# AniruddhaMandal/SS-GNN

Measured on AMD Instinct MI355X. Metric: k_subgraphs_sampled_per_sec, higher is better.
Workload: dtype int64; 1 GPU; c5_er_1m; graphs=1, columns=19999981, k=8, rows_per_gpu=1000000, global_rows=1000000, mode=sample, collate=none (single GPU)

## Files before the change

### include/ugs_mi355.h

```cpp
#ifndef UGS_MI355_H
#define UGS_MI355_H

#include <stdint.h>

#ifdef __cplusplus
extern "C" {
#endif

#define UGS_OK 0
#define UGS_E_INVALID_HANDLE (-1)
#define UGS_E_NO_ROOTS (-2)
#define UGS_E_BAD_MODE (-3)
#define UGS_E_BAD_ARG (-4)
#define UGS_E_NO_DEVICE (-5)
#define UGS_E_HIP (-6)
#define UGS_E_UNSUPPORTED (-7)
#define UGS_E_EDGE_SRC (-8)
#define UGS_E_CAPACITY (-9)

#define UGS_EDGE_LOCAL 0
#define UGS_EDGE_FLAT 1
#define UGS_EDGE_GLOBAL 2
#define UGS_MODE_SAMPLE 0
#define UGS_MODE_GRAPH 1
// ... 37 lines not shown
int ugs_sample_batch_stream(const int64_t *edge_index, int64_t row_stride, int64_t num_cols, const int64_t *ptr,
                            int64_t num_graphs, int m_per_graph, int k, int mode, int seed, int64_t edge_capacity,
                            int64_t *nodes, int64_t *edge_index_out, int64_t *edge_ptr, int64_t *sample_ptr,
                            int64_t *edge_src_global, int64_t *total_edges_out);
int ugs_sample_stream(int64_t handle, int m_per_graph, int k, int edge_mode, int64_t base_offset, int seed,
                      int64_t edge_capacity, int64_t *nodes, int64_t *edge_index_out, int64_t *edge_ptr, int64_t *edge_src,
                      int64_t *total_edges_out);
int ugs_stream_stats(int64_t *early_starts_kept, int64_t *early_starts_discarded);

int ugs_cache_clear(void);
int ugs_cache_stats(int64_t *size, int64_t *hits, int64_t *misses);
int ugs_batch_pass_stats(int64_t *device_plans, int64_t *general_path);
int ugs_set_batch_pass_max_cols(int64_t cols, int64_t *previous_out);
int64_t ugs_batch_pass_max_cols(void);

typedef struct ugs_plan ugs_plan;
int ugs_plan_create_batch(const int64_t *edge_index, int64_t row_stride, int64_t num_cols, const int64_t *ptr,
                          int64_t num_graphs, int k, ugs_plan **plan_out);
int ugs_plan_create_handle(int64_t handle, ugs_plan **plan_out);
int ugs_plan_release(ugs_plan *plan);
int ugs_plan_graph_roots(ugs_plan *plan, int64_t graph, int64_t capacity, int32_t *level, int32_t *num_nodes, int32_t *num_viable,
                         double *prob, int32_t *alias, int32_t *v_self, int32_t *v_alias, int32_t *viable_vi, int32_t *viable_v);
int ugs_plan_twin(ugs_plan *plan, int k, ugs_plan **twin_out);
int ugs_plan_info(const ugs_plan *plan, int k, int64_t *num_graphs, int64_t *num_vertices, int64_t *nnz,
                  int64_t *device_bytes, int *tier);
int ugs_plan_walk(ugs_plan *plan, int m_per_graph, int k, int mode, int64_t extra_node_offset, int seed,
                  int64_t row_begin, int64_t row_count, void *stream, int64_t *d_nodes, int64_t *d_edge_ptr,
                  int64_t *total_edges_host);
int ugs_plan_fill(ugs_plan *plan, int m_per_graph, int k, int mode, int64_t extra_node_offset, int64_t row_begin,
                  int64_t row_count, void *stream, const int64_t *d_nodes, const int64_t *d_edge_ptr,
                  int64_t *d_edge_index, int64_t ld, int64_t *d_edge_src);
int ugs_plan_step(ugs_plan *plan, int m_per_graph, int k, int mode, int64_t extra_node_offset, int seed, int64_t row_begin,
                  int64_t row_count, void *stream, int64_t *d_nodes, int64_t *d_edge_ptr, int64_t *d_edge_index, int64_t ld,
                  int64_t *d_edge_src);
int ugs_plan_set_walk_share(ugs_plan *plan, int percent);
typedef struct ugs_graph ugs_graph;
int ugs_plan_graph_create(ugs_plan *plan, int m_per_graph, int k, int mode, int64_t extra_node_offset, int64_t row_begin,
                          int64_t row_count, int64_t *d_nodes, int64_t *d_edge_ptr, int64_t *d_edge_index, int64_t ld,
                          int64_t *d_edge_src, ugs_graph **graph_out);
int ugs_plan_graph_launch(ugs_graph *graph, int seed, void *stream);
int ugs_plan_graph_destroy(ugs_graph *graph);
int ugs_plan_last_launch(const ugs_plan *plan, char *name_buf, int name_buf_len, int *grid, int *block,
                         int *lds_bytes, int64_t *overflow_rows);

int ugs_collate_layout(int k, int node_bytes, int eidx_bytes, int esrc_bytes, int64_t rows_cap, int64_t edge_cap,
                       int64_t *section_off4, int64_t *msg_bytes);
// ... 62 lines not shown
```

### ss-gnn_amd/csrc/ugs_device.h

```cpp
#pragma once
#include <hip/hip_runtime.h>
#include <stdint.h>

#define UGS_KMAX 32

struct UgsGraphDesc {
    int64_t node_lo;
    int64_t rbase;
    int64_t vbase;
    int64_t viable_base;
    int32_t n;
    int32_t level;
    int32_t n_viable;
    int32_t pad;
};

struct UgsRootRec {
    double prob;
    int32_t alias;
    int32_t v_self;
    int32_t v_alias;
    int32_t pad;
};

struct UgsPlanDev {
    const UgsGraphDesc *graphs;
    const int64_t *rowptr;
    const int2 *adj;
    const int2 *adjf;
    const UgsRootRec *roots;
    const int2 *viable;
    int64_t num_graphs;
    const int2 *prow;
    int32_t prow_shift;
    int32_t prow_first;
};

struct UgsWalkArgs {
    UgsPlanDev plan;
    int32_t m;
    int32_t k;
    int32_t mode;
    int32_t pad;
    int64_t extra_node_off;
    uint64_t seed64;
    const uint64_t *seed_ptr;
    int64_t row_begin;
    int64_t row_count;
    int64_t *nodes;
    uint32_t *counts;
    const int64_t *in_list;
    const uint32_t *in_count;
    int64_t *ovf_list;
    uint32_t *ovf_count;
    uint32_t *gws;
    int64_t gws_words_per_group;
    int64_t gws_groups;
    int32_t gcap;
// ... 31 lines not shown
    int64_t *h_total;
    uint32_t *h_flag;
    uint32_t epoch;
};

struct UgsLaunchInfo {
    const char *name;
    int grid, block, lds_bytes;
};

enum { UGS_TIER_S = 0 , UGS_TIER_M = 1 , UGS_TIER_W = 2 ,
       UGS_TIER_X = 3 , UGS_TIER_V = 4 , UGS_TIER_L = 5 ,
       UGS_TIER_G = 6  };
#define UGS_LDS_TIERS 6
static constexpr int UGS_TIER_CAP[UGS_LDS_TIERS] = {64, 448, 704, 1024, 1408, 2048};
static constexpr int UGS_TIER_LANES[UGS_LDS_TIERS] = {8, 64, 64, 64, 64, 64};
static constexpr int UGS_TIER_HASH_LIMIT[UGS_LDS_TIERS] = {96, 448, 896, 1536, 1792, 3072};
#define UGS_SMALL_CAP 32
#define UGS_WIDE_LANES 16
#define UGS_SMALL_HASH_LIMIT 48

hipError_t ugs_launch_walk(const UgsWalkArgs &a, int tier, int device_cus, int share_percent, hipStream_t s, UgsLaunchInfo *info);
hipError_t ugs_launch_build_prow(const UgsPlanDev &plan, int64_t num_vertices, int2 *prow, int shift, int device_cus, hipStream_t s);
#define UGS_COLLATE_MAX_WORLD 64
hipError_t ugs_launch_collate_unpack(const void *d_msgs, int world, int64_t msg_bytes, const int64_t *row_off, int k, int node_b, int eidx_b,
                                     int esrc_b, int64_t rows_cap, int64_t edge_cap, const int64_t *section_off4, int64_t *d_nodes,
                                     int64_t *d_edge_index, int64_t ld, int64_t *d_edge_ptr, int64_t *d_edge_src, int64_t *d_max_total,
                                     hipStream_t s);
hipError_t ugs_launch_rebase_edge_ptr(const int64_t *in, int64_t *out, int64_t n, int64_t base, hipStream_t s);
#define UGS_BATCH_PASS_MAX_COLS 1000
#define UGS_BATCH_PASS_COLS_CEIL 8192
#define UGS_BATCH_PASS_MAX_N 2048
#define UGS_BATCH_PASS_FUSED_WORK (4ll << 20)
int64_t ugs_batch_pass_fused_work();
hipError_t ugs_launch_batch_pass(const int64_t *d_src, const int64_t *d_dst, int64_t E, const int64_t *d_ptr, int64_t G, int k,
                                 int32_t *d_owner, uint32_t *d_cnt_jminc_jmax, const int64_t *d_rstart, int64_t *d_rowptr, int2 *d_adj,
                                 int2 *d_adjf, int32_t *d_vrank, unsigned long long *d_bump, unsigned long long bump_base, uint32_t epoch, void *h_back,
                                 unsigned long long *d_done, unsigned long long done_base, int64_t max_cols, hipStream_t s);
#define UGS_BP_BACK_CNT(G) ((size_t)(G) * 24)
#define UGS_BP_BACK_FLAG(G) ((size_t)(G) * 36)
#define UGS_BP_BACK_BYTES(G) ((size_t)(G) * 36 + 16)
__host__ __device__ inline unsigned long long ugs_fp_mix(unsigned long long x) {
    x ^= x >> 33; x *= 0xff51afd7ed558ccdull; x ^= x >> 33; x *= 0xc4ceb9fe1a85ec53ull; x ^= x >> 33;
    return x;
}
__host__ __device__ inline void ugs_fp_seed(unsigned long long n, unsigned long long cols, unsigned long long &a, unsigned long long &b) {
// ... 105 lines not shown
```

### ss-gnn_amd/csrc/ugs_host.cpp

```cpp
#include "../../include/ugs_mi355.h"
#include "ugs_device.h"

#include <algorithm>
#include <atomic>
#include <cmath>
#include <cstdio>
#include <cstdlib>
#include <cstring>
#include <chrono>
#include <list>
#include <map>
#include <memory>
#include <mutex>
#include <string>
#include <unordered_map>
#include <thread>
#include <vector>

struct ugs_plan;
namespace { void plan_unref(ugs_plan *p); void arena_release(int dev, int64_t roots_off, int64_t n_roots, int64_t via_off, int64_t n_via); void pin_slot_put(char *p); }

struct UgsEpsLaunch {
    const UgsGraphDesc *graphs; const int64_t *rowptr; const int32_t *nbr; const int32_t *ecs; int64_t num_graphs;
    int32_t m, k, mode, max_attempts; uint64_t seed; double epsilon; int64_t rows;
// ... 850 lines not shown
            if (v >= ptr[g] && v < ptr[g + 1]) { owner[(size_t)j] = (int32_t)g; ++cstart[(size_t)g + 1]; }
        }
        for (int64_t g = 0; g < G; ++g) cstart[(size_t)g + 1] += cstart[(size_t)g];
        cols_of.resize((size_t)cstart[(size_t)G]);
        std::vector<int64_t> wr(cstart.begin(), cstart.end() - 1);
        for (int64_t j = 0; j < E; ++j) if (owner[(size_t)j] >= 0) cols_of[(size_t)wr[(size_t)owner[(size_t)j]]++] = j;
    } else {
        for (int64_t g = 0; g < G; ++g) {
            const int64_t lo = ptr[g], hi = ptr[g + 1];
            for (int64_t j = 0; j < E; ++j) if (src[j] >= lo && src[j] < hi && dst[j] >= lo && dst[j] < hi) cols_of.push_back(j);
            cstart[(size_t)g + 1] = (int64_t)cols_of.size();
        }
    }
}

int ensure_prow(ugs_plan *plan, hipStream_t s) {
    if (plan->dev.prow || plan->prow_failed || plan->nverts <= 0) return UGS_OK;
    if (const char *e = std::getenv("UGS_NO_PROW")) if (e[0] == '1') return UGS_OK;
    double sb = 0;
    for (double x : plan->g_sbdeg) sb = std::max(sb, x);
    int shift = 3;
    while (shift < 6 && (double)((1 << shift) - 1) < sb + 3.0 * std::sqrt(sb) + 1.0) ++shift;
    if (const char *e = std::getenv("UGS_PROW_SHIFT")) { const int f = std::atoi(e); if (f >= 3 && f <= 6) shift = f; }
    const size_t bytes = ((size_t)plan->nverts << shift) * sizeof(int2);
    if (bytes >= ((size_t)1 << 32)) { plan->prow_failed = true; return UGS_OK; }
    if (bytes <= ((size_t)64 << 20)) {
        const std::string keep = t_err;
        if (pool_get(bytes, plan->device, plan->prow) != UGS_OK) { t_err = keep; plan->prow_failed = true; return UGS_OK; }
        plan->prow_pooled = true;
    } else {
        void *p = nullptr;
        if (hipMalloc(&p, bytes) != hipSuccess) { (void)hipGetLastError(); plan->prow_failed = true; return UGS_OK; }
        plan->prow.p = p; plan->prow.bytes = bytes; plan->prow.dev = plan->device;
    }
    HIP_TRY(ugs_launch_build_prow(plan->dev, plan->nverts, static_cast<int2 *>(plan->prow.p), shift, plan->cus, s));
    HIP_TRY(hipStreamSynchronize(s));
    plan->dev.prow = static_cast<const int2 *>(plan->prow.p);
    plan->dev.prow_shift = shift;
    int first = (int)std::ceil((sb + 0.5 * std::sqrt(sb) + 1.0) / 16.0) * 16;
    if (const char *e = std::getenv("UGS_PROW_FIRST")) { const int f = std::atoi(e); if (f >= 1) first = f; }
    plan->dev.prow_first = std::max(1, std::min(first, 1 << shift));
    plan->prow_bytes.store(plan->prow.bytes);
    if (plan->cached) plan_cache_trim();
    return UGS_OK;
}

int ensure(PoolBuf &b, size_t bytes, int dev, ugs_plan *plan) {
    if (b.p && b.bytes >= bytes) return UGS_OK;
    if (b.p && plan && plan->last_valid) HIP_TRY(hipEventSynchronize(plan->last_ev));
    pool_put(b);
    return pool_get(bytes, dev, b);
}

bool capturing(hipStream_t s) {
    hipStreamCaptureStatus st = hipStreamCaptureStatusNone;
    return hipStreamIsCapturing(s, &st) == hipSuccess && st != hipStreamCaptureStatusNone;
}
int plan_enter(ugs_plan *plan, hipStream_t s) {
    if (plan->last_valid && plan->last_stream != s && !capturing(s)) HIP_TRY(hipStreamWaitEvent(s, plan->last_ev, 0));
    return UGS_OK;
}
int plan_leave(ugs_plan *plan, hipStream_t s) {
    if (capturing(s)) return UGS_OK;
    if (!plan->last_ev) HIP_TRY(hipEventCreateWithFlags(&plan->last_ev, hipEventDisableTiming));
    HIP_TRY(hipEventRecord(plan->last_ev, s));
// ... 681 lines not shown
        std::lock_guard<std::mutex> lk(plan->mu);
        if (plan->last_valid) HIP_TRY(hipEventSynchronize(plan->last_ev));
        HIP_TRY(hipMemcpy(&d, plan->dev.graphs + graph, sizeof(d), hipMemcpyDeviceToHost));
    }
    if (level) *level = d.level;
    if (num_nodes) *num_nodes = d.n;
    if (num_viable) *num_viable = d.n_viable;
    if (d.level == 0 && d.n > 0 && (prob || alias || v_self || v_alias)) {
        if (capacity < d.n) return fail(UGS_E_BAD_ARG, "capacity below the graph's vertex count");
        std::vector<UgsRootRec> rec((size_t)d.n);
        HIP_TRY(hipMemcpy(rec.data(), plan->dev.roots + d.vbase, rec.size() * sizeof(UgsRootRec), hipMemcpyDeviceToHost));
        for (int32_t vi = 0; vi < d.n; ++vi) {
            if (prob) prob[vi] = rec[(size_t)vi].prob;
            if (alias) alias[vi] = rec[(size_t)vi].alias;
            if (v_self) v_self[vi] = rec[(size_t)vi].v_self;
            if (v_alias) v_alias[vi] = rec[(size_t)vi].v_alias;
        }
    } else if (d.level > 0 && d.n_viable > 0 && (viable_vi || viable_v)) {
        if (capacity < d.n_viable) return fail(UGS_E_BAD_ARG, "capacity below the viable list's length");
        std::vector<int2> v((size_t)d.n_viable);
        HIP_TRY(hipMemcpy(v.data(), plan->dev.viable + d.viable_base, v.size() * sizeof(int2), hipMemcpyDeviceToHost));
        for (int32_t t = 0; t < d.n_viable; ++t) { if (viable_vi) viable_vi[t] = v[(size_t)t].x; if (viable_v) viable_v[t] = v[(size_t)t].y; }
    }
    return UGS_OK;
}

int ugs_plan_info(const ugs_plan *plan, int k, int64_t *num_graphs, int64_t *num_vertices, int64_t *nnz, int64_t *device_bytes, int *tier) {
    if (!plan) return fail(UGS_E_BAD_ARG, "plan is null");
    if (num_graphs) *num_graphs = plan->G;
    if (num_vertices) *num_vertices = plan->nverts;
    if (nnz) *nnz = plan->nnz;
    if (device_bytes) *device_bytes = (int64_t)(plan->blob_bytes + plan->prow.bytes);
    if (tier) *tier = choose_tier(const_cast<ugs_plan *>(plan), k).first;
    return UGS_OK;
}

static int plan_walk_impl(ugs_plan *plan, int m_per_graph, int k, int mode, int64_t extra_node_offset, int seed, const uint64_t *d_seed_ptr,
                          const uint64_t *d_seeds, int64_t row_begin, int64_t row_count, void *stream, int64_t *d_nodes, int64_t *d_edge_ptr, int64_t *total_edges_host,
                          bool *defer_scan = nullptr, bool poll_total = false);
static int plan_walk_locked(ugs_plan *plan, const TierChoice &tc, int m_per_graph, int k, int mode, int64_t extra_node_offset, int seed,
                            const uint64_t *d_seed_ptr, const uint64_t *d_seeds, int64_t row_begin, int64_t row_count, hipStream_t s, int64_t *d_nodes, int64_t *d_edge_ptr,
                            int64_t *total_edges_host, bool *defer_scan, bool poll_total);


int ugs_plan_walk(ugs_plan *plan, int m_per_graph, int k, int mode, int64_t extra_node_offset, int seed, int64_t row_begin,
                  int64_t row_count, void *stream, int64_t *d_nodes, int64_t *d_edge_ptr, int64_t *total_edges_host) {
// ... 1289 lines not shown
```

### ss-gnn_amd/csrc/ugs_kernels.hip

```cpp
#include "ugs_device.h"
#include <cstdlib>

#define UGS_ALIGNED16 __attribute__((aligned(16)))

#ifdef UGS_STAMPS
__device__ unsigned long long ugs_stamp_buffer[32];
#define ST_ ws.ST
#define STAMP_DECL unsigned long long st_t0 = 0
#define STAMP_BEGIN() do { __builtin_amdgcn_sched_barrier(0); st_t0 = __builtin_amdgcn_s_memtime(); __builtin_amdgcn_sched_barrier(0); } while (0)
#define STAMP_END(i) do { __builtin_amdgcn_sched_barrier(0); const unsigned long long t1_ = __builtin_amdgcn_s_memtime(); \
    if ((threadIdx.x & 63) == 0) { atomicAdd(&ST_[i], t1_ - st_t0); atomicAdd(&ST_[16 + (i)], 1ull); } st_t0 = __builtin_amdgcn_s_memtime(); __builtin_amdgcn_sched_barrier(0); } while (0)
#define STAMP_SUB_BEGIN() __builtin_amdgcn_sched_barrier(0); const unsigned long long sti_ = __builtin_amdgcn_s_memtime(); __builtin_amdgcn_sched_barrier(0)
#define STAMP_SUB_END_OF(parent, i) do { __builtin_amdgcn_sched_barrier(0); const unsigned long long t1_ = __builtin_amdgcn_s_memtime(); \
    if ((threadIdx.x & 63) == 0) { atomicAdd(&ST_[i], t1_ - sti_); atomicAdd(&ST_[parent], sti_ - t1_); atomicAdd(&ST_[16 + (i)], 1ull); } __builtin_amdgcn_sched_barrier(0); } while (0)
#define STAMP_SUB_END(i) STAMP_SUB_END_OF(2, i)
#else
#define STAMP_DECL
#define STAMP_SUB_BEGIN() do {} while (0)
#define STAMP_SUB_END(i) do {} while (0)
#define STAMP_SUB_END_OF(parent, i) do {} while (0)
#define STAMP_BEGIN() do {} while (0)
#define STAMP_END(i) do {} while (0)
#endif

// ... 379 lines not shown
    const uint32_t above = size - 1u - g.below(mates);
    const uint32_t first = valid ? (uint32_t)__builtin_ctzll(mates) : (uint32_t)g.lane;
    const uint32_t lead = (valid && first == (uint32_t)g.lane) ? size : 0u;
    const uint32_t incl = g.template prefix_incl_first<MAXN>(lead);
    const uint32_t run = n_valid - incl;
    const uint32_t start = (uint32_t)__builtin_amdgcn_ds_bpermute((int)(first << 2), (int)run);
    return start + above;
}

template <int MAXN = 64>
__device__ __forceinline__ void stage_mat_reg(const Work<LdsSpace> &ws, const Grp<64> &g, const uint16_t *OLD, uint16_t *NEW,
                                              uint32_t n_old, uint32_t B, uint32_t M, uint32_t S) {
    const uint32_t t = (uint32_t)g.lane;
    const bool valid = t < B;
    uint32_t pos = t;
    if (n_old) { const uint32_t o = OLD[t]; pos = t < n_old ? o : t; }
    const uint32_t key = ws.D[pos];
    const uint32_t rank = rank_in_registers<MAXN>(g, valid, mod_stage(key, B, M, S), ws.TBL, B, B);
    if (valid) NEW[rank] = (uint16_t)pos;
    LdsSpace::sync();
}

template <int MAXN = 64>
__device__ __forceinline__ Pick stage_final_reg(const Work<LdsSpace> &ws, const Grp<64> &g, const uint16_t *OLD, uint32_t n_old,
                                                uint32_t L, uint32_t B, uint32_t M, uint32_t S, uint32_t rsel) {
    const uint32_t t = (uint32_t)g.lane;
    const bool valid = t < L;
    uint32_t pos = t;
    if (n_old) { const uint32_t o = OLD[t]; pos = t < n_old ? o : t; }
    const uint32_t key = ws.D[pos];
    const uint32_t rank = rank_in_registers<MAXN>(g, valid, mod_stage(key, B, M, S), ws.TBL, B, L);
    const uint64_t hm = __ballot(rank == rsel) & (~0ull >> (64u - L));
    const int src = __builtin_ctzll(hm);
    return Pick{g.bcast(key, src), g.bcast(pos, src)};
}

struct Rank2 { uint32_t r0, r1; };
__device__ __forceinline__ void mates2_by_table(uint32_t *TBL, const Grp<64> &g, bool valid1, uint32_t bk0, uint32_t bk1, uint32_t B,
                                                uint64_t &m00, uint64_t &m01, uint64_t &m10, uint64_t &m11) {
    uint4 *T4 = reinterpret_cast<uint4 *>(TBL);
    for (uint32_t i = (uint32_t)g.lane; i < B; i += 64) T4[i] = make_uint4(0u, 0u, 0u, 0u);
    LdsSpace::sync();
    unsigned long long *T8 = reinterpret_cast<unsigned long long *>(TBL);
    const unsigned long long bit = 1ull << g.lane;
    atomicOr(&T8[2u * bk0], bit);
    if (valid1) atomicOr(&T8[2u * bk1 + 1u], bit);
    LdsSpace::sync();
    const uint4 a = T4[bk0], b = T4[bk1];
    m00 = ((uint64_t)a.y << 32) | a.x; m01 = ((uint64_t)a.w << 32) | a.z;
    m10 = ((uint64_t)b.y << 32) | b.x; m11 = ((uint64_t)b.w << 32) | b.z;
}
__device__ __forceinline__ Rank2 rank2_from_mates(const Grp<64> &g, bool valid1, uint64_t m00, uint64_t m01, uint64_t m10, uint64_t m11) {
    const uint64_t gt = ~1ull << g.lane;
    const uint32_t lane = (uint32_t)g.lane;
// ... 543 lines not shown
template <int GS, class SP, bool ADD, bool STG>
__device__ __forceinline__ bool scan_row(const Work<SP> &ws, const Grp<GS> &g, const int2 *adj, uint32_t v,
                                         uint32_t root_vi, uint32_t size, uint32_t &c, uint32_t &hcount,
                                         uint32_t &ecount, uint32_t r0, uint32_t r1, StageCtx &sc) {
    for (uint32_t base = r0; base < r1; base += GS) {
        const uint32_t p = base + (uint32_t)g.lane;
        int2 e = UGS_NO_ENTRY;
        if (p < r1) e = adj[p];
        if (!scan_chunk<GS, SP, ADD, STG>(ws, g, v, root_vi, size, c, hcount, ecount, sc, e, p)) return false;
    }
    return true;
}

__device__ __forceinline__ int2 prow_entry(const UgsPlanDev &P, int64_t vrow, int lane) {
    const uint32_t off = (((uint32_t)vrow << P.prow_shift) + (uint32_t)lane) << 3;
    return *reinterpret_cast<const int2 *>(reinterpret_cast<const char *>(P.prow) + off);
}
__device__ __forceinline__ int2 load_prow(const UgsPlanDev &P, int64_t vrow, int lane) {
    int2 e = make_int2(0, 0);
    if (lane < P.prow_first) e = prow_entry(P, vrow, lane);
    return e;
}

template <class SP, bool ADD, bool STG, bool SON = false>
__device__ __forceinline__ bool scan_prow(const Work<SP> &ws, const Grp<64> &g, const UgsPlanDev &P, uint32_t v,
                                          uint32_t root_vi, uint32_t size, uint32_t &c, uint32_t &hcount,
                                          uint32_t &ecount, int2 e0, int64_t vrow, StageCtx &sc) {
    const uint32_t deg = g.bcast((uint32_t)e0.x, 0);
    const uint32_t start = g.bcast((uint32_t)e0.y, 0);
    const uint32_t inl = (1u << P.prow_shift) - 1u;
    const uint32_t n0 = deg < inl ? deg : inl;
    if (n0 >= (uint32_t)P.prow_first) {
        if (g.lane >= P.prow_first && g.lane <= (int)n0) e0 = prow_entry(P, vrow, g.lane);
    }
    if ((uint32_t)(g.lane - 1) >= n0) e0 = UGS_NO_ENTRY;
    uint32_t n0a = n0, n0b = n0;
    asm volatile("" : "+s"(n0a));
    asm volatile("" : "+s"(n0b));
    if constexpr (ADD) {
        if (__builtin_expect(hcount + deg <= ws.hlimit && c + deg <= ws.cap, 1)) {
            if (n0a) scan_chunk<64, SP, true, STG, false, SON>(ws, g, v, root_vi, size, c, hcount, ecount, sc, e0, start + (uint32_t)g.lane - 1u);
            if (__builtin_expect(deg > inl, 0)) {
                const uint32_t r1 = start + deg;
                for (uint32_t base = start + inl; base < r1; base += 64) {
                    const uint32_t p = base + (uint32_t)g.lane;
                    int2 e = UGS_NO_ENTRY;
// ... 146 lines not shown
    } else {
        const uint32_t idx = mod64_root(rng.next(), (uint32_t)gd.n_viable);
        vr = P.viable[gd.viable_base + idx];
    }
    __builtin_amdgcn_sched_barrier(0);
    {
        uint4 *H4 = reinterpret_cast<uint4 *>(ws.HK);
        const uint32_t n4 = (ws.hmask + 1u) >> 2;
        for (uint32_t s = g.lane; s < n4; s += GS) H4[s] = make_uint4(kEmpty, kEmpty, kEmpty, kEmpty);
    }
    if (gd.level == 0) {
        const bool self = u < rr.prob;
        root_vi = g.uni(self ? j : (uint32_t)rr.alias);
        root_v = g.uni((uint32_t)(self ? rr.v_self : rr.v_alias));
    } else {
        root_vi = g.uni((uint32_t)vr.x);
        root_v = g.uni((uint32_t)vr.y);
    }
    uint32_t r0 = 0, r1 = 0;
    int2 e0 = make_int2(0, 0);
    uint32_t v = root_v;
    if constexpr (PAD) e0 = load_prow(P, gd.vbase + v, g.lane);
    else { r0 = g.uni((uint32_t)P.rowptr[gd.rbase + v]); r1 = g.uni((uint32_t)P.rowptr[gd.rbase + v + 1]); }
    SP::sync();
    if (g.lane == 0) { ws.HK[hash_slot(root_v, ws.hmask)] = root_v | kInS; SV[0] = root_v; }
    SP::sync();
    uint32_t size = 1, c = 0, hcount = 1, ecount = 0;
    int nvalid = 0;
    STAMP_END(0);
    for (int step = 0;; ++step) {
        Grp<GS> g = g_;
        if constexpr (GS == 64) asm volatile("" : "+v"(g.lane));
#ifdef UGS_PAD
        {
            uint32_t pad_;
#if UGS_PAD == 1
#define UGS_PAD1 asm volatile("s_mov_b32 %0, 0" : "=s"(pad_));
#elif UGS_PAD == 2
#define UGS_PAD1 asm volatile("s_mov_b32 %0, 0x12345678" : "=s"(pad_));
#elif UGS_PAD == 3
#define UGS_PAD1 asm volatile("v_mov_b32_e32 %0, 0" : "=v"(pad_));
#elif UGS_PAD == 4
#define UGS_PAD1 asm volatile("v_mov_b32_e64 %0, 0" : "=v"(pad_));
#elif UGS_PAD == 5
#define UGS_PAD1 asm volatile("s_cmp_eq_u32 0, 0\ns_cbranch_scc0 ugs_pad_%=\nugs_pad_%=:" : "=s"(pad_) : : "scc");
#elif UGS_PAD == 6
// ... 4 lines not shown
#define UGS_PAD1 asm volatile("s_nop 1" : "=s"(pad_));
#else
#define UGS_PAD1 asm volatile("s_waitcnt lgkmcnt(0)" : "=s"(pad_));
#endif
#define UGS_PAD8 UGS_PAD1 UGS_PAD1 UGS_PAD1 UGS_PAD1 UGS_PAD1 UGS_PAD1 UGS_PAD1 UGS_PAD1
            UGS_PAD8 UGS_PAD8 UGS_PAD8 UGS_PAD8 UGS_PAD8 UGS_PAD8 UGS_PAD8 UGS_PAD8
#undef UGS_PAD8
#undef UGS_PAD1
        }
#endif
        bool ok;
        if (step < k - 1) {
            if constexpr (PAD) ok = scan_prow<SP, true, STG, UNI>(ws, g, P, v, root_vi, size, c, hcount, ecount, e0, gd.vbase + v, sc);
            else ok = scan_row<GS, SP, true, STG>(ws, g, P.adj, v, root_vi, size, c, hcount, ecount, r0, r1, sc);
        } else {
            if constexpr (PAD) ok = scan_prow<SP, false, STG, UNI>(ws, g, P, v, root_vi, size, c, hcount, ecount, e0, gd.vbase + v, sc);
            else ok = scan_row<GS, SP, false, STG>(ws, g, P.adj, v, root_vi, size, c, hcount, ecount, r0, r1, sc);
        }
        STAMP_END(1);
        if (!ok) return false;
        if (step >= k - 1 || c == 0) break;
        const uint32_t rsel = g.uni(mod64_by<sizeof(typename SP::TW) == 4, sizeof(typename SP::TW) == 4 && GS == 64>(rng.next(), c));
        STAMP_END(4);
        const Pick pick = select_any<GS, MAXPER>(ws, g, c, rsel, nvalid);
        const uint32_t w = pick.w;
        if constexpr (PAD) {
            e0 = load_prow(P, gd.vbase + w, g.lane);
        } else {
            r0 = (uint32_t)P.rowptr[gd.rbase + w];
            r1 = (uint32_t)P.rowptr[gd.rbase + w + 1];
            r0 = g.uni(r0); r1 = g.uni(r1);
        }
        STAMP_END(2);
        uint32_t q = pick.q;
        if constexpr (sizeof(typename SP::TW) != 4) {
            for (uint32_t t0 = 0; t0 < c && q == c; t0 += 4 * GS) {
                uint32_t x[4];
#pragma unroll
                for (int u = 0; u < 4; ++u) { const uint32_t t = t0 + u * GS + g.lane; x[u] = (t < c) ? ws.D[t] : kEmpty; }
#pragma unroll
                for (int u = 0; u < 4; ++u) {
                    const uint64_t mk = g.ballot(x[u] == w);
                    if (mk && q == c) q = t0 + u * GS + (uint32_t)(__ffsll((long long)mk) - 1);
                }
            }
        }
        STAMP_END(7);
// ... 199 lines not shown
            if (g.lane == 0 && a.ovf_list) { uint32_t pos = atomicAdd(a.ovf_count, 1u); a.ovf_list[pos] = row_rel; }
        }
    }
}

__global__ __launch_bounds__(256) void ugs_build_prow(UgsPlanDev P, int64_t num_vertices, int2 *prow, int shift) {
    const int64_t idx = (int64_t)blockIdx.x * 256 + threadIdx.x;
    const int64_t R = idx >> shift;
    if (R >= num_vertices) return;
    const int l = (int)(idx & ((1 << shift) - 1));
    int64_t lo = 0, hi = P.num_graphs - 1;
    while (lo < hi) {
        const int64_t mid = (lo + hi + 1) >> 1;
        if (P.graphs[mid].vbase <= R) lo = mid; else hi = mid - 1;
    }
    const int64_t rb = P.graphs[lo].rbase, v = R - P.graphs[lo].vbase;
    const int64_t start = P.rowptr[rb + v], deg = P.rowptr[rb + v + 1] - start;
    int2 e = make_int2(0, 0);
    if (l == 0) e = make_int2((int)deg, (int)start);
    else if (l - 1 < deg) e = P.adj[start + l - 1];
    prow[idx] = e;
}

template <bool SEEDS>
__global__ __launch_bounds__(64) void ugs_walk_global(UgsWalkArgs a) {
    __shared__ uint32_t SV[UGS_KMAX];
    Grp<64> g;
    g.init();
    uint32_t *base = a.gws + (int64_t)blockIdx.x * a.gws_words_per_group;
    Work<GlbSpace> ws;
    auto al4 = [](int64_t x) { return (x + 3) & ~3ll; };
    ws.TBL = (unsigned long long *)base;
    ws.D = base + 2 * al4(a.gbcap);
    ws.ORD = ws.D + al4(a.gcap);
    ws.AUX = ws.ORD + al4(a.gpcap);
    ws.HK = ws.AUX + al4(a.gcap);
    ws.cap = (uint32_t)a.gcap;
    ws.hmask = (uint32_t)a.ghs - 1u;
    ws.hlimit = (uint32_t)a.ghs / 4u * 3u;
#ifdef UGS_STAMPS
    __shared__ unsigned long long stamps[32];
    ws.ST = stamps;
#endif
    const int64_t total = a.in_list ? (int64_t)*a.in_count : a.row_count;
    for (int64_t it = blockIdx.x; it < total; it += gridDim.x) {
        const int64_t row_rel = a.in_list ? a.in_list[it] : it;
// ... 416 lines not shown
    case UGS_TIER_W: return launch_lds<64, 704, 64>(a, cus, part(12), s, info, "ugs_walk_lds<64,704>");
    case UGS_TIER_X: return launch_lds<64, 1024, 64>(a, cus, part(8), s, info, "ugs_walk_lds<64,1024>");
    case UGS_TIER_V: return launch_lds<64, 1408, 64>(a, cus, part(6), s, info, "ugs_walk_lds<64,1408>");
    case UGS_TIER_L: return launch_lds<64, 2048, 64>(a, cus, part(4), s, info, "ugs_walk_lds<64,2048>");
    default: {
        int64_t grid = a.gws_words_per_group > 0 ? a.gws_groups : 0;
        if (grid < 1) return hipErrorInvalidValue;
        if (a.seeds) hipLaunchKernelGGL(ugs_walk_global<true>, dim3((unsigned)grid), dim3(64), 0, s, a);
        else hipLaunchKernelGGL(ugs_walk_global<false>, dim3((unsigned)grid), dim3(64), 0, s, a);
        if (info) { info->name = "ugs_walk_global"; info->grid = (int)grid; info->block = 64; info->lds_bytes = UGS_KMAX * 4; }
        return hipGetLastError();
    }
    }
}

hipError_t ugs_launch_build_prow(const UgsPlanDev &plan, int64_t num_vertices, int2 *prow, int shift, int cus, hipStream_t s) {
    (void)cus;
    const int64_t total = num_vertices << shift;
    if (total <= 0) return hipSuccess;
    hipLaunchKernelGGL(ugs_build_prow, dim3((unsigned)((total + 255) / 256)), dim3(256), 0, s, plan, num_vertices, prow, shift);
    return hipGetLastError();
}

hipError_t ugs_launch_scan(const uint32_t *counts, int64_t rows, int64_t *edge_ptr, int64_t *block_tmp, hipStream_t s, int64_t *h_total,
                           uint32_t *h_flag, uint32_t epoch) {
    if (rows <= 0) { return hipMemsetAsync(edge_ptr, 0, sizeof(int64_t), s); }
    const ScanSignal sg{h_total, h_flag, epoch};
    if (rows <= (int64_t)2 * kScanWide * kScanPer) {
        hipLaunchKernelGGL(ugs_scan_small, dim3(1), dim3(kScanWide), 0, s, counts, rows, edge_ptr, sg);
        return hipGetLastError();
    }
    const int64_t nb = (rows + kScanTile - 1) / kScanTile;
    hipLaunchKernelGGL(ugs_scan_partials, dim3((unsigned)nb), dim3(kScanBlock), 0, s, counts, rows, block_tmp);
    if (nb <= 4096) {
        hipLaunchKernelGGL(ugs_scan_final_sum, dim3((unsigned)nb), dim3(kScanBlock), 0, s, counts, rows, (const int64_t *)block_tmp, edge_ptr, sg);
        return hipGetLastError();
    }
    hipLaunchKernelGGL(ugs_scan_block_sums, dim3(1), dim3(kScanBlock), 0, s, block_tmp, nb);
    hipLaunchKernelGGL(ugs_scan_final, dim3((unsigned)nb), dim3(kScanBlock), 0, s, counts, rows, (const int64_t *)block_tmp, edge_ptr, sg);
    return hipGetLastError();
}

template <int BLOCK>
__global__ __launch_bounds__(BLOCK) void ugs_fill_staged(UgsFillArgs a) {
    constexpr int GS = 16, GROUPS = BLOCK / GS;
    const int lane = (int)threadIdx.x & (GS - 1), gib = (int)threadIdx.x / GS;
// ... 69 lines not shown
```

### ss-gnn_amd/ugs_sampler/_lib.py

```python
import ctypes as C
import os

_HERE = os.path.dirname(os.path.abspath(__file__))
_CSRC = os.path.join(os.path.dirname(_HERE), "csrc")
LIB_PATH = os.environ.get("UGS_MI355_LIB", os.path.join(_CSRC, "libugs_mi355.so"))

i64p = C.POINTER(C.c_int64)
vp = C.c_void_p


def _load():
    if not os.path.exists(LIB_PATH):
        raise ImportError(
            f"ugs_sampler: {LIB_PATH} is missing -- build the HIP library first "
            f"(python {os.path.join(_CSRC, 'build.py')}  or  python -c 'import __graft_entry__ as g; g.build()'). "
            "This sampler has no CPU fallback.")
    L = C.CDLL(LIB_PATH)
    L.ugs_last_error.restype = C.c_char_p
    L.ugs_version.restype = C.c_char_p
    sig = {
        "ugs_device_count": [C.POINTER(C.c_int)],
        "ugs_set_device": [C.c_int],
        "ugs_set_stream": [vp, C.c_int],
        "ugs_create_preproc": [vp, C.c_int64, C.c_int64, C.c_int64, C.c_int, i64p],
# ... 20 lines not shown
        "ugs_eps_sample_graphs_begin": [vp, C.c_int64, C.c_int64, vp, C.c_int64, C.c_int, C.c_int, C.c_int, vp, C.c_double, vp,
                                        C.POINTER(vp), i64p],
        "ugs_uniform_sample_batch_begin": [vp, C.c_int64, C.c_int64, vp, C.c_int64, C.c_int, C.c_int, C.c_int, C.c_uint64,
                                           C.POINTER(vp), i64p],
        "ugs_uniform_sample_batch_finish": [vp, vp, vp, vp, vp, vp, C.c_int],
        "ugs_rwr_sample_batch_begin": [vp, C.c_int64, C.c_int64, vp, C.c_int64, C.c_int, C.c_int, C.c_int, C.c_uint64, C.c_double,
                                       C.POINTER(vp), i64p],
        "ugs_rwr_sample_batch_finish": [vp, vp, vp, vp, vp, vp, C.c_int],
        "ugs_uniform_sample_graphs_begin": [vp, C.c_int64, C.c_int64, vp, C.c_int64, C.c_int, C.c_int, C.c_int, vp, vp,
                                            C.POINTER(vp), i64p],
        "ugs_rwr_sample_graphs_begin": [vp, C.c_int64, C.c_int64, vp, C.c_int64, C.c_int, C.c_int, C.c_int, vp, C.c_double, vp,
                                        C.POINTER(vp), i64p],
        "ugs_cache_clear": [],
        "ugs_cache_stats": [i64p, i64p, i64p],
        "ugs_batch_pass_stats": [i64p, i64p],
        "ugs_set_batch_pass_max_cols": [C.c_int64, i64p],
        "ugs_uniform_set_max_vertices": [C.c_int, C.POINTER(C.c_int)],
        "ugs_uniform_set_mask_vertices": [C.c_int, C.POINTER(C.c_int)],
        "ugs_plan_create_batch": [vp, C.c_int64, C.c_int64, vp, C.c_int64, C.c_int, C.POINTER(vp)],
        "ugs_plan_create_handle": [C.c_int64, C.POINTER(vp)],
        "ugs_plan_release": [vp],
        "ugs_plan_graph_roots": [vp, C.c_int64, C.c_int64, C.POINTER(C.c_int32), C.POINTER(C.c_int32), C.POINTER(C.c_int32)] + [vp] * 6,
        "ugs_plan_twin": [vp, C.c_int, C.POINTER(vp)],
        "ugs_plan_info": [vp, C.c_int, i64p, i64p, i64p, i64p, C.POINTER(C.c_int)],
        "ugs_plan_walk": [vp, C.c_int, C.c_int, C.c_int, C.c_int64, C.c_int, C.c_int64, C.c_int64, vp, vp, vp, i64p],
        "ugs_plan_fill": [vp, C.c_int, C.c_int, C.c_int, C.c_int64, C.c_int64, C.c_int64, vp, vp, vp, vp, C.c_int64, vp],
        "ugs_plan_step": [vp, C.c_int, C.c_int, C.c_int, C.c_int64, C.c_int, C.c_int64, C.c_int64, vp, vp, vp, vp, C.c_int64, vp],
        "ugs_plan_graph_create": [vp, C.c_int, C.c_int, C.c_int, C.c_int64, C.c_int64, C.c_int64, vp, vp, vp, C.c_int64, vp, C.POINTER(vp)],
        "ugs_plan_graph_launch": [vp, C.c_int, vp],
        "ugs_plan_graph_destroy": [vp],
        "ugs_collate_layout": [C.c_int, C.c_int, C.c_int, C.c_int, C.c_int64, C.c_int64, i64p, i64p],
        "ugs_collate_unpack": [vp, C.c_int, i64p, C.c_int, C.c_int, C.c_int, C.c_int, C.c_int64, C.c_int64, vp, vp, C.c_int64, vp, vp, vp, vp],
        "ugs_plan_set_walk_share": [vp, C.c_int],
        "ugs_plan_set_timing": [vp, C.c_int],
        "ugs_plan_get_timing": [vp, C.POINTER(C.c_double), i64p],
        "ugs_plan_last_launch": [vp, C.c_char_p, C.c_int, C.POINTER(C.c_int), C.POINTER(C.c_int), C.POINTER(C.c_int), i64p],
        "ugs_wl_hash": [vp, vp, C.c_int64, C.c_int64, vp, C.c_int64, C.c_int, C.c_int, vp, vp],
        "ugs_wl_hash_labeled": [vp, vp, C.c_int64, C.c_int64, vp, C.c_int64, C.c_int, C.c_int, vp, C.c_int64, vp, vp],
        "ugs_wl_feature_labels": [vp, C.c_int64, C.c_int64, C.c_int64, vp],
        "ugs_wl_lookup": [vp, vp, C.c_int64, vp, vp, C.c_int64, C.c_int64, vp],
    }
    for name, argtypes in sig.items():
        fn = getattr(L, name)
        fn.argtypes = argtypes
        fn.restype = C.c_int
    L.ugs_batch_pass_max_cols.argtypes = []
# ... 17 lines not shown
```

Measured before the change: 222.0 million k-subgraphs/s.

## Precompute per-vertex first-step pick table to skip initial selection in walks

Adds a per-vertex 64-entry uint16 table, built once at plan setup by a new kernel, that records the candidate count after the root, the final rank-to-position mapping and the stage orders for roots with at most 59 candidates. During the walk's first step the kernel reads this record and picks directly instead of running select_any and its staged ranking. This removes the first-step ranking work but adds a 128-byte-per-vertex table load per root and a sizable one-time build cost and memory footprint.

```diff
diff --git a/include/ugs_mi355.h b/include/ugs_mi355.h
--- a/include/ugs_mi355.h
+++ b/include/ugs_mi355.h
@@ -83,6 +83,7 @@
 int ugs_plan_graph_roots(ugs_plan *plan, int64_t graph, int64_t capacity, int32_t *level, int32_t *num_nodes, int32_t *num_viable,
                          double *prob, int32_t *alias, int32_t *v_self, int32_t *v_alias, int32_t *viable_vi, int32_t *viable_v);
 int ugs_plan_twin(ugs_plan *plan, int k, ugs_plan **twin_out);
+int ugs_plan_first_pick_table(ugs_plan *plan, void *host_out, int64_t out_bytes, int64_t *table_bytes);
 int ugs_plan_info(const ugs_plan *plan, int k, int64_t *num_graphs, int64_t *num_vertices, int64_t *nnz,
                   int64_t *device_bytes, int *tier);
 int ugs_plan_walk(ugs_plan *plan, int m_per_graph, int k, int mode, int64_t extra_node_offset, int seed,
diff --git a/ss-gnn_amd/csrc/ugs_device.h b/ss-gnn_amd/csrc/ugs_device.h
--- a/ss-gnn_amd/csrc/ugs_device.h
+++ b/ss-gnn_amd/csrc/ugs_device.h
@@ -34,6 +34,7 @@
     const int2 *prow;
     int32_t prow_shift;
     int32_t prow_first;
+    const uint16_t *fpick;
 };
 
 struct UgsWalkArgs {
@@ -111,6 +112,9 @@
 
 hipError_t ugs_launch_walk(const UgsWalkArgs &a, int tier, int device_cus, int share_percent, hipStream_t s, UgsLaunchInfo *info);
 hipError_t ugs_launch_build_prow(const UgsPlanDev &plan, int64_t num_vertices, int2 *prow, int shift, int device_cus, hipStream_t s);
+#define UGS_FPICK_ENTRIES 64
+#define UGS_FPICK_MAX_C 59
+hipError_t ugs_launch_build_fpick(const UgsPlanDev &plan, int64_t num_vertices, uint16_t *fpick, int device_cus, hipStream_t s);
 #define UGS_COLLATE_MAX_WORLD 64
 hipError_t ugs_launch_collate_unpack(const void *d_msgs, int world, int64_t msg_bytes, const int64_t *row_off, int k, int node_b, int eidx_b,
                                      int esrc_b, int64_t rows_cap, int64_t edge_cap, const int64_t *section_off4, int64_t *d_nodes,
diff --git a/ss-gnn_amd/csrc/ugs_host.cpp b/ss-gnn_amd/csrc/ugs_host.cpp
--- a/ss-gnn_amd/csrc/ugs_host.cpp
+++ b/ss-gnn_amd/csrc/ugs_host.cpp
@@ -896,8 +896,13 @@
     int shift = 3;
     while (shift < 6 && (double)((1 << shift) - 1) < sb + 3.0 * std::sqrt(sb) + 1.0) ++shift;
     if (const char *e = std::getenv("UGS_PROW_SHIFT")) { const int f = std::atoi(e); if (f >= 3 && f <= 6) shift = f; }
-    const size_t bytes = ((size_t)plan->nverts << shift) * sizeof(int2);
-    if (bytes >= ((size_t)1 << 32)) { plan->prow_failed = true; return UGS_OK; }
+    const size_t row_bytes = ((size_t)plan->nverts << shift) * sizeof(int2);
+    if (row_bytes >= ((size_t)1 << 32)) { plan->prow_failed = true; return UGS_OK; }
+    size_t fp_bytes = (size_t)plan->nverts * UGS_FPICK_ENTRIES * sizeof(uint16_t);
+    if (fp_bytes >= ((size_t)1 << 32)) fp_bytes = 0;
+    if (const char *e = std::getenv("UGS_NO_FIRST_PICK")) if (e[0] == '1') fp_bytes = 0;
+    const size_t fp_off = (row_bytes + 127) & ~(size_t)127;
+    const size_t bytes = fp_bytes ? fp_off + fp_bytes : row_bytes;
     if (bytes <= ((size_t)64 << 20)) {
         const std::string keep = t_err;
         if (pool_get(bytes, plan->device, plan->prow) != UGS_OK) { t_err = keep; plan->prow_failed = true; return UGS_OK; }
@@ -915,6 +920,12 @@
     if (const char *e = std::getenv("UGS_PROW_FIRST")) { const int f = std::atoi(e); if (f >= 1) first = f; }
     plan->dev.prow_first = std::max(1, std::min(first, 1 << shift));
     plan->prow_bytes.store(plan->prow.bytes);
+    if (fp_bytes) {
+        uint16_t *fp = reinterpret_cast<uint16_t *>(static_cast<char *>(plan->prow.p) + fp_off);
+        HIP_TRY(ugs_launch_build_fpick(plan->dev, plan->nverts, fp, plan->cus, s));
+        HIP_TRY(hipStreamSynchronize(s));
+        plan->dev.fpick = fp;
+    }
     if (plan->cached) plan_cache_trim();
     return UGS_OK;
 }
@@ -1642,6 +1653,18 @@
         HIP_TRY(hipMemcpy(v.data(), plan->dev.viable + d.viable_base, v.size() * sizeof(int2), hipMemcpyDeviceToHost));
         for (int32_t t = 0; t < d.n_viable; ++t) { if (viable_vi) viable_vi[t] = v[(size_t)t].x; if (viable_v) viable_v[t] = v[(size_t)t].y; }
     }
+    return UGS_OK;
+}
+
+int ugs_plan_first_pick_table(ugs_plan *plan, void *host_out, int64_t out_bytes, int64_t *table_bytes) {
+    if (!plan) return fail(UGS_E_BAD_ARG, "plan is null");
+    std::lock_guard<std::mutex> lk(plan->mu);
+    const int64_t bytes = plan->dev.fpick ? plan->nverts * (int64_t)(UGS_FPICK_ENTRIES * sizeof(uint16_t)) : 0;
+    if (table_bytes) *table_bytes = bytes;
+    if (!host_out || !bytes) return UGS_OK;
+    if (out_bytes < bytes) return fail(UGS_E_BAD_ARG, "buffer smaller than the first-pick table");
+    HIP_TRY(hipSetDevice(plan->device));
+    HIP_TRY(hipMemcpy(host_out, plan->dev.fpick, (size_t)bytes, hipMemcpyDeviceToHost));
     return UGS_OK;
 }
 
diff --git a/ss-gnn_amd/csrc/ugs_kernels.hip b/ss-gnn_amd/csrc/ugs_kernels.hip
--- a/ss-gnn_amd/csrc/ugs_kernels.hip
+++ b/ss-gnn_amd/csrc/ugs_kernels.hip
@@ -425,14 +425,21 @@
 }
 
 template <int MAXN = 64>
+__device__ __forceinline__ uint32_t final_rank_reg(const Work<LdsSpace> &ws, const Grp<64> &g, const uint16_t *OLD, uint32_t n_old,
+                                                   uint32_t L, uint32_t B, uint32_t M, uint32_t S, uint32_t &pos, uint32_t &key) {
+    const uint32_t t = (uint32_t)g.lane;
+    const bool valid = t < L;
+    pos = t;
+    if (n_old) { const uint32_t o = OLD[t]; pos = t < n_old ? o : t; }
+    key = ws.D[pos];
+    return rank_in_registers<MAXN>(g, valid, mod_stage(key, B, M, S), ws.TBL, B, L);
+}
+
+template <int MAXN = 64>
 __device__ __forceinline__ Pick stage_final_reg(const Work<LdsSpace> &ws, const Grp<64> &g, const uint16_t *OLD, uint32_t n_old,
                                                 uint32_t L, uint32_t B, uint32_t M, uint32_t S, uint32_t rsel) {
-    const uint32_t t = (uint32_t)g.lane;
-    const bool valid = t < L;
-    uint32_t pos = t;
-    if (n_old) { const uint32_t o = OLD[t]; pos = t < n_old ? o : t; }
-    const uint32_t key = ws.D[pos];
-    const uint32_t rank = rank_in_registers<MAXN>(g, valid, mod_stage(key, B, M, S), ws.TBL, B, L);
+    uint32_t pos, key;
+    const uint32_t rank = final_rank_reg<MAXN>(ws, g, OLD, n_old, L, B, M, S, pos, key);
     const uint64_t hm = __ballot(rank == rsel) & (~0ull >> (64u - L));
     const int src = __builtin_ctzll(hm);
     return Pick{g.bcast(key, src), g.bcast(pos, src)};
@@ -1022,6 +1029,22 @@
     return e;
 }
 
+constexpr uint32_t kFpB0 = ChainAt<0>::B, kFpB1 = ChainAt<1>::B;
+constexpr uint32_t kFpOrdLanes = kFpB0 + kFpB1;
+constexpr uint32_t kFpCountLane = UGS_FPICK_MAX_C;
+static_assert(ChainAt<0>::O == 0u && ChainAt<1>::O >= kFpB0 && ChainAt<2>::O >= ChainAt<1>::O + kFpB1, "stage 0 and 1 orders at the head of ORD");
+static_assert(ChainAt<2>::B == UGS_FPICK_MAX_C && kFpOrdLanes <= 64u && UGS_FPICK_MAX_C < UGS_FPICK_ENTRIES && UGS_FPICK_MAX_C <= 0xFF,
+              "a record describes the roots whose final is at most the 59-bucket stage, positions in one byte");
+__device__ __forceinline__ uint32_t fpick_ord_word(uint32_t lane) { return lane < kFpB0 ? lane : lane - kFpB0 + ChainAt<1>::O; }
+__device__ __forceinline__ uint32_t fpick_pack(uint32_t final_or_count, uint32_t ord) { return final_or_count | (ord << 8); }
+__device__ __forceinline__ uint32_t fpick_final(uint32_t entry) { return entry & 0xFFu; }
+__device__ __forceinline__ uint32_t fpick_ord(uint32_t entry) { return entry >> 8; }
+
+__device__ __forceinline__ uint32_t load_fpick(const UgsPlanDev &P, int64_t vrow, int lane) {
+    const uint32_t off = (((uint32_t)vrow << 6) + (uint32_t)lane) << 1;
+    return *reinterpret_cast<const uint16_t *>(reinterpret_cast<const char *>(P.fpick) + off);
+}
+
 template <class SP, bool ADD, bool STG, bool SON = false>
 __device__ __forceinline__ bool scan_prow(const Work<SP> &ws, const Grp<64> &g, const UgsPlanDev &P, uint32_t v,
                                           uint32_t root_vi, uint32_t size, uint32_t &c, uint32_t &hcount,
@@ -1214,6 +1237,8 @@
     uint32_t v = root_v;
     if constexpr (PAD) e0 = load_prow(P, gd.vbase + v, g.lane);
     else { r0 = g.uni((uint32_t)P.rowptr[gd.rbase + v]); r1 = g.uni((uint32_t)P.rowptr[gd.rbase + v + 1]); }
+    uint32_t fprec = 0u;
+    if constexpr (PAD && STG) { if (P.fpick) fprec = load_fpick(P, gd.vbase + v, g.lane); }
     SP::sync();
     if (g.lane == 0) { ws.HK[hash_slot(root_v, ws.hmask)] = root_v | kInS; SV[0] = root_v; }
     SP::sync();
@@ -1264,7 +1289,20 @@
         if (step >= k - 1 || c == 0) break;
         const uint32_t rsel = g.uni(mod64_by<sizeof(typename SP::TW) == 4, sizeof(typename SP::TW) == 4 && GS == 64>(rng.next(), c));
         STAMP_END(4);
-        const Pick pick = select_any<GS, MAXPER>(ws, g, c, rsel, nvalid);
+        Pick pick;
+        bool picked = false;
+        if constexpr (PAD && STG) {
+            if (fpick_final(g.bcast(fprec, (int)kFpCountLane)) == c && step == 0) {
+                const uint32_t q = fpick_final(g.bcast(fprec, (int)rsel));
+                if ((uint32_t)g.lane < kFpOrdLanes) ws.ORD[fpick_ord_word((uint32_t)g.lane)] = (uint16_t)fpick_ord(fprec);
+                nvalid = chain_index_below_lanes(c, g_.chain);
+                pick = Pick{g.uni(ws.D[q]), q};
+                fprec = 0u;
+                picked = true;
+                SP::sync();
+            }
+        }
+        if (!picked) pick = select_any<GS, MAXPER>(ws, g, c, rsel, nvalid);
         const uint32_t w = pick.w;
         if constexpr (PAD) {
             e0 = load_prow(P, gd.vbase + w, g.lane);
@@ -1510,6 +1548,94 @@
     prow[idx] = e;
 }
 
+template <int STAGE>
+__device__ __forceinline__ uint32_t fpick_final_rank(const Work<LdsSpace> &ws, const Grp<64> &g, uint32_t c, uint32_t &pos) {
+    using C = ChainAt<STAGE>;
+    uint32_t key;
+    return final_rank_reg<(int)(C::B < 64u ? C::B : 64u)>(ws, g, ws.ORD + C::OOLD, C::NOLD, c, C::B, C::M, C::S, pos, key);
+}
+__global__ __launch_bounds__(64) void ugs_build_fpick(UgsPlanDev P, int64_t num_vertices, uint16_t *fpick) {
+    constexpr int CAP = 448;
+    using Cfg = TierCfg<CAP>;
+    __shared__ __attribute__((aligned(16))) uint32_t lds[Cfg::WORDS];
+    Grp<64> g;
+    g.init();
+    g.chain = chain_lane_const<Cfg::NSTAGE>(g.lane);
+    Work<LdsSpace> ws;
+    ws.D = lds;
+    ws.ORD = reinterpret_cast<uint16_t *>(ws.D + CAP);
+    ws.AUX = nullptr;
+    ws.TBL = ws.D + CAP + Cfg::ORDW;
+    ws.HK = ws.TBL + Cfg::BCAP_A;
+    ws.cap = CAP;
+    ws.hmask = Cfg::HS - 1;
+    ws.hlimit = Cfg::HLIMIT;
+#ifdef UGS_STAMPS
+    __shared__ unsigned long long stamps[32];
+    ws.ST = stamps;
+#endif
+    StageCtx sc;
+    sc.EL = nullptr; sc.ne = 0u; sc.on = false; sc.onm = 0ull;
+    for (int64_t R = blockIdx.x; R < num_vertices; R += gridDim.x) {
+        int64_t lo = 0, hi = P.num_graphs - 1;
+        while (lo < hi) {
+            const int64_t mid = (lo + hi + 1) >> 1;
+            if (P.graphs[mid].vbase <= R) lo = mid; else hi = mid - 1;
+        }
+        const int64_t rb = P.graphs[lo].rbase;
+        const uint32_t v = (uint32_t)(R - P.graphs[lo].vbase);
+        int2 e0 = load_prow(P, R, g.lane);
+        {
+            uint4 *H4 = reinterpret_cast<uint4 *>(ws.HK);
+            for (uint32_t s = g.lane; s < (uint32_t)Cfg::HS / 4u; s += 64) H4[s] = make_uint4(kEmpty, kEmpty, kEmpty, kEmpty);
+        }
+        const uint32_t deg = g.bcast((uint32_t)e0.x, 0), start = g.bcast((uint32_t)e0.y, 0);
+        uint32_t rec = 0u;
+        if (deg) {
+            const uint32_t w1 = (uint32_t)P.adj[start].x;
+            const uint32_t r0 = (uint32_t)P.rowptr[rb + w1], r1 = (uint32_t)P.rowptr[rb + w1 + 1];
+            uint32_t root_vi = 0u;
+            bool found = false;
+            for (uint32_t base = r0; base < r1 && !found; base += 64) {
+                const uint32_t p = base + (uint32_t)g.lane;
+                int2 e = UGS_NO_ENTRY;
+                if (p < r1) e = P.adj[p];
+                const uint64_t mk = __ballot((uint32_t)e.x == v);
+                if (mk) { root_vi = g.bcast((uint32_t)e.y, __builtin_ctzll(mk)); found = true; }
+            }
+            LdsSpace::sync();
+            if (g.lane == 0) ws.HK[hash_slot(v, ws.hmask)] = v | kInS;
+            LdsSpace::sync();
+            uint32_t c = 0u, hcount = 1u, ecount = 0u;
+            const bool ok = found && scan_prow<LdsSpace, true, false>(ws, g, P, v, root_vi, 1u, c, hcount, ecount, e0, R, sc);
+            if (ok && c >= 1u && c <= (uint32_t)UGS_FPICK_MAX_C) {
+                uint32_t pos, rank;
+                if (c > ChainAt<1>::B) {
+                    mat_at<64, CAP / 64, 0>(ws, g);
+                    mat_at<64, CAP / 64, 1>(ws, g);
+                    rank = fpick_final_rank<2>(ws, g, c, pos);
+                } else if (c > ChainAt<0>::B) {
+                    mat_at<64, CAP / 64, 0>(ws, g);
+                    rank = fpick_final_rank<1>(ws, g, c, pos);
+                } else {
+                    rank = fpick_final_rank<0>(ws, g, c, pos);
+                }
+                LdsSpace::sync();
+                if ((uint32_t)g.lane < c) ws.TBL[rank] = pos;
+                LdsSpace::sync();
+                const uint32_t lane = (uint32_t)g.lane;
+                uint32_t lo8 = lane < c ? ws.TBL[lane] : 0u;
+                if (lane == kFpCountLane) lo8 = c;
+                uint32_t hi8 = 0u;
+                if (lane < kFpOrdLanes && c > (lane < kFpB0 ? kFpB0 : kFpB1)) hi8 = ws.ORD[fpick_ord_word(lane)];
+                rec = fpick_pack(lo8, hi8);
+                LdsSpace::sync();
+            }
+        }
+        fpick[R * UGS_FPICK_ENTRIES + g.lane] = (uint16_t)rec;
+    }
+}
+
 template <bool SEEDS>
 __global__ __launch_bounds__(64) void ugs_walk_global(UgsWalkArgs a) {
     __shared__ uint32_t SV[UGS_KMAX];
@@ -1972,6 +2098,16 @@
     return hipGetLastError();
 }
 
+hipError_t ugs_launch_build_fpick(const UgsPlanDev &plan, int64_t num_vertices, uint16_t *fpick, int cus, hipStream_t s) {
+    if (num_vertices <= 0) return hipSuccess;
+    if (!plan.prow) return hipErrorInvalidValue;
+    if (cus <= 0) cus = 256;
+    int64_t grid = (int64_t)cus * UGS_BLOCKS_M;
+    if (grid > num_vertices) grid = num_vertices;
+    hipLaunchKernelGGL(ugs_build_fpick, dim3((unsigned)grid), dim3(64), 0, s, plan, num_vertices, fpick);
+    return hipGetLastError();
+}
+
 hipError_t ugs_launch_scan(const uint32_t *counts, int64_t rows, int64_t *edge_ptr, int64_t *block_tmp, hipStream_t s, int64_t *h_total,
                            uint32_t *h_flag, uint32_t epoch) {
     if (rows <= 0) { return hipMemsetAsync(edge_ptr, 0, sizeof(int64_t), s); }
diff --git a/ss-gnn_amd/ugs_sampler/_lib.py b/ss-gnn_amd/ugs_sampler/_lib.py
--- a/ss-gnn_amd/ugs_sampler/_lib.py
+++ b/ss-gnn_amd/ugs_sampler/_lib.py
@@ -66,6 +66,7 @@
         "ugs_plan_release": [vp],
         "ugs_plan_graph_roots": [vp, C.c_int64, C.c_int64, C.POINTER(C.c_int32), C.POINTER(C.c_int32), C.POINTER(C.c_int32)] + [vp] * 6,
         "ugs_plan_twin": [vp, C.c_int, C.POINTER(vp)],
+        "ugs_plan_first_pick_table": [vp, vp, C.c_int64, i64p],
         "ugs_plan_info": [vp, C.c_int, i64p, i64p, i64p, i64p, C.POINTER(C.c_int)],
         "ugs_plan_walk": [vp, C.c_int, C.c_int, C.c_int, C.c_int64, C.c_int, C.c_int64, C.c_int64, vp, vp, vp, i64p],
         "ugs_plan_fill": [vp, C.c_int, C.c_int, C.c_int, C.c_int64, C.c_int64, C.c_int64, vp, vp, vp, vp, C.c_int64, vp],
```

New measurement: 226.1 million k-subgraphs/s (median of 6 runs). 1.8% higher.
